# SomeBottle/LinearProgramming

Measured on AMD Instinct MI355X. Metric: Simplex pivots/sec + HBM GB/s fraction, dense m=16384×n=32768 fp64, 1/2/4/8 GPU, higher is better.
Workload: dtype f64

## Files before the change

include/lpg.h:

```cpp
#ifndef LPG_H
#define LPG_H

#include <stddef.h>
#include <stdint.h>

#ifdef __cplusplus
extern "C" {
#endif

#define LPG_OK           0
#define LPG_ERR_ARG     -1
#define LPG_ERR_DEVICE  -2
#define LPG_ERR_OOM     -3
#define LPG_ERR_STATE   -4
#define LPG_ERR_COMM    -5

#define LPG_RUNNING      0
#define LPG_OPTIMAL      1
#define LPG_UNBOUNDED    2
#define LPG_INFEASIBLE   3
#define LPG_ITER_LIMIT   4
#define LPG_NUMERIC      5

#define LPG_RULE_DANTZIG 0
// ... 23 lines not shown
} lpg_result;

typedef struct {
    int64_t m, ncols, ld;
    int64_t row0, nrows;
    int32_t world, rank, device;
    int32_t nobj;
    int32_t defer_k;
    int32_t pivot_wg;
    double  bytes_per_pivot;
    int32_t exchange;
    int32_t column_trade;
    int32_t residency_fallbacks;
    int32_t region;
    int32_t region_recoveries;
} lpg_info_t;

typedef struct {
    double  update_ms;
    double  select_ms;
    double  comm_ms;
    int64_t update_count;
    double  update_bytes;
} lpg_timing;

typedef struct {
    void *user;
    int (*allgather)(void *user, const void *send, void *recv, size_t bytes_per_rank);
    int (*allreduce_sum_f64)(void *user, double *buf, size_t count);
} lpg_host_comm_ops;
// ... 145 lines not shown
```

linearprogramming_amd/_lib.py:

```python
from __future__ import annotations

import ctypes
import os
import sys

_HERE = os.path.dirname(os.path.abspath(__file__))
LIB_PATH = os.path.join(_HERE, "liblpg.so")

OK, ERR_ARG, ERR_DEVICE, ERR_OOM, ERR_STATE, ERR_COMM = 0, -1, -2, -3, -4, -5
RUNNING, OPTIMAL, UNBOUNDED, INFEASIBLE, ITER_LIMIT, NUMERIC = 0, 1, 2, 3, 4, 5
STATUS_NAMES = {0: "RUNNING", 1: "OPTIMAL", 2: "UNBOUNDED", 3: "INFEASIBLE", 4: "ITER_LIMIT", 5: "NUMERIC"}
RULE_DANTZIG, RULE_BLAND = 0, 1
GEN_DENSE, GEN_DEGENERATE, GEN_ARTIFICIAL, GEN_DUAL = 0, 1, 2, 3
FLAG_NO_LOG = 0x1
FLAG_NO_SKIP = 0x2
FLAG_BIG_M = 0x4
FLAG_EAGER = 0x8
DEFER_MAX = 128
BATCH_TIER_LDS, BATCH_TIER_GLOBAL = 0, 1
BATCH_MAX_DIM = 8192
BRANCH_MOST_FRACTIONAL, BRANCH_FIRST = 0, 1
BATCH_MAX_CUTS = 1024

c_double_p = ctypes.POINTER(ctypes.c_double)
# ... 2 lines not shown
c_int8_p = ctypes.POINTER(ctypes.c_int8)


class Result(ctypes.Structure):
    _fields_ = [("status", ctypes.c_int32), ("rule", ctypes.c_int32), ("pivots", ctypes.c_int64),
                ("objective", ctypes.c_double), ("entering", ctypes.c_int64), ("leaving", ctypes.c_int64)]


class Info(ctypes.Structure):
    _fields_ = [("m", ctypes.c_int64), ("ncols", ctypes.c_int64), ("ld", ctypes.c_int64),
                ("row0", ctypes.c_int64), ("nrows", ctypes.c_int64),
                ("world", ctypes.c_int32), ("rank", ctypes.c_int32), ("device", ctypes.c_int32),
                ("nobj", ctypes.c_int32), ("defer_k", ctypes.c_int32), ("pivot_wg", ctypes.c_int32),
                ("bytes_per_pivot", ctypes.c_double), ("exchange", ctypes.c_int32), ("column_trade", ctypes.c_int32),
                ("residency_fallbacks", ctypes.c_int32), ("region", ctypes.c_int32),
                ("region_recoveries", ctypes.c_int32)]


class Timing(ctypes.Structure):
    _fields_ = [("update_ms", ctypes.c_double), ("select_ms", ctypes.c_double),
                ("comm_ms", ctypes.c_double), ("update_count", ctypes.c_int64), ("update_bytes", ctypes.c_double)]


class BatchInfo(ctypes.Structure):
    _fields_ = [("count", ctypes.c_int64), ("m", ctypes.c_int64), ("ncols", ctypes.c_int64), ("ld", ctypes.c_int64),
                ("tier", ctypes.c_int32), ("chunk", ctypes.c_int32), ("lds_bytes", ctypes.c_int64),
                ("log_capacity", ctypes.c_int64), ("nobj", ctypes.c_int32), ("pad", ctypes.c_int32)]


class BatchShape(ctypes.Structure):
    _fields_ = [("m", ctypes.c_int64), ("ncols", ctypes.c_int64), ("ld", ctypes.c_int64),
# ... 219 lines not shown
```

linearprogramming_amd/csrc/lpg_block.hip:

```cpp
#include <hip/hip_runtime.h>
#include <math.h>
#include <stdint.h>

#include <algorithm>
#include <atomic>

#include "lpg_device.h"
#include "lpg_internal.h"

namespace lpg {

typedef unsigned u4 __attribute__((ext_vector_type(4)));

namespace {

constexpr int kNT = 256;
constexpr int kMaxWG = 256;
constexpr int kPer = kMaxWG / 64;
constexpr int kRecPMax = 5;
constexpr int kRecR = 2;
constexpr int kMaxLds = 150 * 1024;
constexpr long long kSpinTicks = 200000000ll;
constexpr int kSweepSleep = 1;

// ... 347 lines not shown
    int ncin;
    Xch X;
    uint32_t xtag0;
    const double *Cs0;
    double *Cs1;
    Defer D;
    u4 *rec;
    uint32_t tag0;
    int nwg, cw, rw, ks;
    uint32_t cl;
    int xcd1;
    const int32_t *live;
    int64_t nlive;
    const int64_t *bcol0;
    int nsp, cwx;
};

template <int RULE, int NOBJ, bool MR, int KB, bool REG>
__global__ __launch_bounds__(kNT, 1) void k_pivot_block(BlockArgs a) {
    static_assert(!REG || NOBJ == 1, "region mode: one objective row");
    constexpr bool B2 = KB > 64;
    constexpr int WS = B2 ? 104 : 72;
    constexpr bool KDR = RULE != RULE_BLAND && NOBJ == 1;
    constexpr int GDR = KDR ? 0 : 2;
    constexpr int NGP = 2 + (KDR ? 0 : 1) + (NOBJ == 2 ? 1 : 0);
    constexpr bool RPIV = !MR && RULE != RULE_BLAND;
    constexpr int NGR = RPIV ? 1 : kRecR;
    static_assert(NGP < kRecPMax, "pricing records (nwg * NGP + 1 granules) exceed their reservation");
    constexpr bool PK1 = NOBJ == 1;
    constexpr bool PKD = PK1 && !KDR;
// ... 400 lines not shown
                }
                if (hc) pq = __longlong_as_double((long long)ld_sys64(xch_row(a.X, a.X.rank, xpar, owner, g.ld) + c));
            }
            if (wg == 0 && tid == 0) {
                D.lv[q] = lvv;
                D.basis[r] = kt;
            }
        }
        if (REG && actnow) {
            pql = (MR && !own) ? __longlong_as_double((long long)ld_sys64(xch_row(a.X, a.X.rank, xpar, xowner, g.ld) +
                                                                          (uint32_t)bc0))
                               : x / piv;
            sPt[q] = pql;
            cobl = cobjR;
            actq = q;
        }
        if (hc) {
            sPt[q] = pq;
            st_wt(D.Pbuf + (int64_t)q * g.ld + c, pq);
            if (NOBJ == 2) dM = fma(-cobjM, pq, dM);
            dR = fma(-cobjR, pq, dR);
            price_one<RULE>(pb, dM, dR, lj, g, c);
            pb.pad = (int32_t)c;
        }
        LPG_BPH(t, 10);
        pb = block_argmin_pp<RULE, kNT / 64, false>(pb);
        LPG_BPH(t, 11);
        if (tid == 0) {
            uint64_t h = ~0ull;
            uint32_t l = ~0u;
            if (pb.j >= 0) {
                h = RULE == RULE_BLAND ? 0ull
                                       : (((uint64_t)(uint32_t)pb.cls << 63) |
                                          (~(uint64_t)__double_as_longlong(pb.v) & 0x7fffffffffffffffull));
// ... 401 lines not shown
    hipLaunchKernelGGL(k_region_build, dim3(1), dim3(1024), 0, (hipStream_t)L.stream, st, basis, inv, g.m, g.ncols,
                       g.ld, mark, live, bcol0, nlive, tlive);
    return hipGetLastError() == hipSuccess ? 0 : -1;
}

int launch_region_check(const Launch &L, const Geo &g, const int64_t *basis, const int32_t *inv, int *ok) {
    const int64_t rows = g.nloc + g.nobj;
    hipLaunchKernelGGL(k_region_check, dim3((unsigned)((rows + 63) / 64), (unsigned)((g.m + 255) / 256)), dim3(256), 0,
                       (hipStream_t)L.stream, g.T, g, basis, inv, ok);
    return hipGetLastError() == hipSuccess ? 0 : -1;
}

int launch_pivot_block(const Launch &L, const Geo &g, int rule, DevState *st, int s0, int q0, int n, Cand *part,
                       int ncand, const Cand *cin, int ncin, const double *Cs0, double *Cs1, const Defer &D,
                       void *rec, uint32_t tag0, int nwg, int cw, int rw, int ks, size_t lds, uint32_t cl,
                       const Xch *X, uint32_t xtag0, const RegionArgs *R) {
    if (n < 1 || q0 < 0 || q0 + n > ks || ks > 96 || nwg < 1 || nwg > kMaxWG || ncand < nwg || cl < 1) return -1;
    if (X && (X->world < 1 || X->world > 64 || X->nblk < nwg || X->nx < 1)) return -1;
    if (!R && ((int64_t)nwg * cw < ((g.ncols + 1) & ~(int64_t)1) || (int64_t)nwg * rw < g.nloc)) return -1;
    if (R && (g.nobj != 1 || (int64_t)nwg * cw < R->nlive || (int64_t)nwg * rw < g.nloc ||
              (int64_t)nwg * R->nsp < ks || R->cwx != cw + R->nsp + 1 || R->cwx > kNT || !R->live || !R->bcol0))
        return -1;
    if (g.nobj != 1 && g.nobj != 2) return -1;
    BlockArgs a;
    a.T = g.T;
    a.g = g;
    a.st = st;
    a.s0 = s0;
    a.q0 = q0;
    a.n = n;
    a.part = part;
// ... 5 lines not shown
    a.Cs0 = Cs0;
    a.Cs1 = Cs1;
    a.D = D;
    a.rec = (u4 *)rec;
    a.tag0 = tag0;
    a.nwg = nwg;
    a.cw = cw;
    a.rw = rw;
    a.ks = ks;
    a.cl = cl;
    a.live = R ? R->live : nullptr;
    a.nlive = R ? R->nlive : 0;
    a.bcol0 = R ? R->bcol0 : nullptr;
    a.nsp = R ? R->nsp : 0;
    a.cwx = R ? R->cwx : cw;
    hipStream_t stream = (hipStream_t)L.stream;
    static const bool xcd1_on = [] {
        const char *e = getenv("LPG_PIVOT_XCD1");
        return !(e && e[0] == '0');
    }();

    int dev = 0;
    if (hipGetDevice(&dev) != hipSuccess || dev < 0 || dev >= 64) return -1;
    static std::atomic<int> cus_of[64];
    int cus = cus_of[dev].load(std::memory_order_relaxed);
    if (cus == 0) {
        if (hipDeviceGetAttribute(&cus, hipDeviceAttributeMultiprocessorCount, dev) != hipSuccess) cus = -1;
        cus_of[dev].store(cus, std::memory_order_relaxed);
    }
    a.xcd1 = (xcd1_on && !X && cus >= 8 * 32 && nwg <= cus / 8) ? 1 : 0;
// ... 44 lines not shown
```

linearprogramming_amd/csrc/lpg_ctx.hip:

```cpp
#include <hip/hip_runtime.h>
#include <rccl/rccl.h>

#include <dlfcn.h>
#include <unistd.h>
#include <math.h>
#include <stdarg.h>
#include <stdio.h>
#include <stdlib.h>
#include <string.h>

#include <algorithm>
#include <cmath>
#include <vector>

#include "../../include/lpg.h"
#include "lpg_internal.h"

using namespace lpg;

namespace {

thread_local char g_err[512];

struct TimingRing {
// ... 37 lines not shown
    int skip_cfg = 1;
    bool no_reorder_cfg = false;
    bool signed_zeros = false;
    bool nonfinite = false;
    int pb_nwg = 0, pb_cw = 0, pb_rw = 0;
    size_t pb_lds = 0;
    bool reg = false;
    bool reg_valid = false;
    bool units_known = false;
    RegionGeo rg{};
    int32_t *live = nullptr, *mark = nullptr;
    int32_t *tlive = nullptr;
    bool block_region = false;
    bool tlive_on = true;
    bool move_unit = true;
    int64_t *bcol0 = nullptr;
    int *rok = nullptr;
    void *rec = nullptr;
    uint32_t tag = 0;
    uint32_t pb_launch = 0;
    int64_t lost = 0;
    int res_fallbacks = 0;
    int reg_recoveries = 0;
    char *xbuf = nullptr;
    int64_t xbytes = 0, xoffF = 0, xoffC = 0, xoffG = 0;
    int xnblk = 0, xnx = 0;
    bool xuncached = false;
    char **xbase = nullptr;
    std::vector<void *> xpeer;
    bool xmode = false;
// ... 231 lines not shown
        default: break;
    }
    return 0;
}

#endif

static int flush_launch(lpg_ctx *c) {
    int rc;
    const bool re = reorders(c);
#ifdef LPG_TEST_HOOKS
    if (c->inject_flush >= 0 && c->nflush == c->inject_flush && (rc = inject_pending_fault(c))) return rc;
#endif
    c->nflush++;
    const int unit = (c->block_region && c->reg_valid && c->move_unit) ? 1 : 0;
    if (launch_swap_plan(lau(c), geo(c), c->st, defer_of(c, 0), c->colmap, c->inv, c->pairs, re ? 1 : 0, c->defer_k) ||
        (re && launch_move_cols(lau(c), geo(c), c->st, defer_of(c, 0), c->pairs, unit)))
        return fail(c, LPG_ERR_DEVICE, "swap plan launch failed");
#ifdef LPG_TEST_HOOKS
    if (c->inject_rbad >= 0 && c->nflush == c->inject_rbad + 1)
        HIPCHK(c, hipMemsetAsync(&c->st->rbad, 0x01, sizeof(uint32_t), c->stream));
#endif
    if (c->timing && ((rc = timing_mark(c, 0)) || (rc = timing_mark(c, 1)))) return rc;
    const int32_t *tl = (c->block_region && c->reg_valid && re && c->tlive_on && c->skip) ? c->tlive : nullptr;
    c->block_region = false;
    if (launch_flush_main(lau(c), geo(c), c->st, defer_of(c, 0), c->pend, c->skip, c->flush_variant, c->flush_xcd, tl))
        return fail(c, LPG_ERR_DEVICE, "flush launch failed");
    if (c->timing && (rc = timing_mark(c, 2, 2))) return rc;
    if (launch_flush_tail(lau(c), geo(c), c->st, defer_of(c, 0), c->pend, !re))
        return fail(c, LPG_ERR_DEVICE, "flush launch failed");
    if (re) {
        const Defer D = defer_of(c, 0);
        if (launch_fill_cols(lau(c), geo(c), c->pairs, c->st, &D, flush_kmax_supported(c->defer_k),
                             c->reg ? c->bcol0 : nullptr))
            return fail(c, LPG_ERR_DEVICE, "fill launch failed");
        c->permuted = true;
    }
    c->pend = 0;
    return 0;
}

static int materialize(lpg_ctx *c) {
    if (c->defer_k == 0 || c->pend == 0) return 0;
    return flush_launch(c);
// ... 179 lines not shown
        if (mr) {
            ncand = std::max(ncand, nwg);
            ncin = c->x_from_cand ? cand_per_rank(c) * c->world : nwg;
            if (c->x_from_cand) cin = c->cand;
            X.base = c->xbase;
            X.world = c->world;
            X.rank = c->rank;
            X.nblk = c->xnblk;
            X.nx = c->xnx;
            X.from_cand = 0;
            X.tag = c->xtag;
            X.offF = c->xoffF;
            X.offC = c->xoffC;
            X.offG = c->xoffG;
        }
        const bool ok = reg ? launch_pivot_block(lau(c), g, rule, c->st, s0, c->pend, n, c->part, ncand, cin, ncin,
                                                 c->C[s0], c->C[s1], defer_of(c, c->pend), c->rec, c->tag, c->rg.nwg,
                                                 c->rg.cw, c->rg.rw, c->defer_k, c->rg.lds, c->pb_launch + 1,
                                                 mr ? &X : nullptr, c->xtag, &R) == 0
                            : launch_pivot_block(lau(c), g, rule, c->st, s0, c->pend, n, c->part, ncand, cin, ncin,
                                                 c->C[s0], c->C[s1], defer_of(c, c->pend), c->rec, c->tag, c->pb_nwg,
                                                 c->pb_cw, c->pb_rw, c->defer_k, c->pb_lds, c->pb_launch + 1,
                                                 mr ? &X : nullptr, c->xtag) == 0;
        if (!ok)
            return fail(c, LPG_ERR_DEVICE, "pivot block launch failed");
        if (reg) c->block_region = true;
        c->pb_launch++;
        if (mr) {
            c->xtag += (uint32_t)n;
            c->x_from_cand = false;
        }
        c->tag += (uint32_t)n;
        c->pend += n;
        c->par = s1;
        c->enq += n;
        npiv -= n;
        if (c->pend == c->defer_k) {
            int rc = flush_launch(c);
            if (rc) return rc;
        }
    }
// ... 178 lines not shown
    return 0;
}

static int recover_region(lpg_ctx *c, const DevState &h) {
    c->reg_recoveries++;
    c->lost += std::max<int64_t>(c->enq - h.pivots, 0);
    c->enq = h.pivots;
    c->pend = (int)h.npend;
    c->booted = false;
    c->reg_valid = false;
    HIPCHK(c, hipMemsetAsync(&c->st->stall, 0, sizeof(int64_t), c->stream));
    return 0;
}

static int pending_fault(lpg_ctx *c, const DevState &h) {
    static const char *const what[] = {"?", "npend", "kq", "lv", "rq"};
    const int64_t w = h.stall_info[0] >= 1 && h.stall_info[0] <= 4 ? h.stall_info[0] : 0;
    c->poisoned = true;
    return fail(c, LPG_ERR_STATE,
                "pending block inconsistent at the flush (%s[%lld] = %lld, npend %lld): the loop was stopped with "
                "NUMERIC instead of indexing with it; the constraint rows were not brought up to date",
                what[w], (long long)h.stall_info[1], (long long)h.stall_info[2], (long long)h.stall_info[3]);
}

static int usable(lpg_ctx *c) {
    if (!c->poisoned) return 0;
    return fail(c, LPG_ERR_STATE, "context unusable: an earlier flush refused an inconsistent pending block, so the "
                "basis and the constraint rows disagree; reload the rows and the basis (lpg_load_rows, lpg_set_basis) or "
                "regenerate (lpg_generate) the LP");
}

static int read_result(lpg_ctx *c, lpg_result *out, int rule) {
// ... 34 lines not shown
    }
    return 0;
}

static int reset_state(lpg_ctx *c) {
    DevState h;
    memset(&h, 0, sizeof h);
    h.logcap = c->logcap;
    h.last_k = h.last_r = -1;
    HIPCHK(c, hipMemcpyAsync(c->st, &h, sizeof h, hipMemcpyHostToDevice, c->stream));
    HIPCHK(c, hipStreamSynchronize(c->stream));
    c->booted = false;
    c->par = 0;
    c->enq = 0;
    c->pend = 0;
    c->touched_mark = 0;
    c->pb_launch = 0;
    c->lost = 0;
    return 0;
}

static void graph_drop(lpg_ctx *c);

static int ensure_log(lpg_ctx *c, int64_t need) {
    if (c->flags & LPG_FLAG_NO_LOG) return 0;
    if (need <= c->logcap) return 0;
    graph_drop(c);
    int64_t cap = std::max<int64_t>(need, 2 * c->logcap);
    int64_t *nk = nullptr, *nr = nullptr;
    HIPCHK(c, hipStreamSynchronize(c->stream));
// ... 107 lines not shown
            static const char *const names[] = {"", "npend", "kq", "lv", "rq", "ahead"};
            for (int u = 1; u <= 5; u++)
                if (!strcmp(w, names[u])) c->inject_what = u;
            c->inject_flush = c->inject_what ? f : -1;
        }
    }
    if (const char *rb = getenv("LPG_TEST_REGION_BAD")) c->inject_rbad = atoi(rb);
#endif
    const char *fv = getenv("LPG_FLUSH_KERNEL");
    c->flush_variant = fv ? (fv[0] == 'w' ? 1 : fv[0] == 'm' ? 0 : -1) : -1;
    const char *ft = getenv("LPG_FLUSH_TLIVE");
    c->tlive_on = !(ft && ft[0] == '0');
    {
        const char *mu = getenv("LPG_MOVE_UNIT");
        c->move_unit = !(mu && mu[0] == '0');
    }
    const char *fx = getenv("LPG_FLUSH_XCD");
    c->flush_xcd = -1;
    if (fx && fx[0] == '0') c->flush_xcd = 0;
    if (fx && fx[0] == '1') c->flush_xcd = 1;
    if (fx && fx[0] == 'h' && (fx[1] == '1' || fx[1] == '2' || fx[1] == '4' || fx[1] == '8')) c->flush_xcd = 10 + (fx[1] - '0');
    int rc;
    if ((rc = use_device(c))) { lpg_destroy(c); return rc; }
    const int64_t rows = c->nloc + c->nobj;
    const Geo g = geo(c);
    c->npp = price_blocks(g);
    const int64_t maxloc = (m + world - 1) / world + c->nobj;
    c->nsel = (int)std::min<int64_t>((maxloc + kBlock - 1) / kBlock, kMaxSelBlocks);
    c->npp_d = pivot_d_blocks(g, 0, c->pivot_nt);
    c->nsel_d = world == 1 ? pivot_d_blocks(g, 1, c->pivot_nt) : (int)((maxloc + 255) / 256);
// ... 308 lines not shown
    o->row0 = c->row0;
    o->nrows = c->nloc;
    o->world = c->world;
    o->rank = c->rank;
    o->device = c->device;
    o->nobj = (int32_t)c->nobj;
    o->defer_k = c->defer_k;
    const bool pb = (c->persist && !has_comm(c)) || (c->persist_x && c->xmode);
    o->pivot_wg = pb ? (c->reg ? c->rg.nwg : c->pb_nwg) : 0;
    o->bytes_per_pivot = 16.0 * (double)(c->nloc + c->nobj) * (double)c->ncols;
    o->exchange = c->xmode ? (c->xuncached ? 2 : 1) : 0;
    o->column_trade = reorders(c) ? 1 : 0;
    o->residency_fallbacks = c->res_fallbacks;
    o->region_recoveries = c->reg_recoveries;
    o->region = (o->pivot_wg > 0 && c->reg) ? 1 : 0;
    return 0;
}

int lpg_load_rows(lpg_ctx *c, int64_t row0, int64_t nrows, const double *rows, int64_t ld) {
    if (!c || !rows || row0 < 0 || nrows < 0 || row0 + nrows > c->m + c->nobj || ld < c->ncols)
        return fail(c, LPG_ERR_ARG, "lpg_load_rows: bad arguments");
    int rc;
    if ((rc = use_device(c)) || (rc = canonicalize(c))) return rc;
    {
        bool sz = false, nf = false;
        for (int64_t i = 0; i < nrows; i++) {
            const double *row = rows + i * ld;
            for (int64_t j = 0; j < c->ncols; j++) {
                const double v = row[j];
                nf |= !std::isfinite(v);
// ... 91 lines not shown
    c->nact = nact;
    c->booted = false;
    graph_drop(c);
    return 0;
}

int lpg_generate(lpg_ctx *c, int64_t n, uint64_t seed, int kind) {
    if (!c || n < 1 || c->ncols != n + c->m + 1 || kind < LPG_GEN_DENSE || kind > LPG_GEN_DUAL)
        return fail(c, LPG_ERR_ARG, "lpg_generate: need ncols == n + m + 1 and a known kind");
    int rc;
    if ((rc = use_device(c))) return rc;
    if (c->colmap && (launch_iota(lau(c), c->colmap, c->ld) || launch_iota(lau(c), c->inv, c->ld)))
        return fail(c, LPG_ERR_DEVICE, "iota launch failed");
    c->permuted = false;
    c->pend = 0;
    if (launch_generate(lau(c), geo(c), n, seed, kind, c->basis)) return fail(c, LPG_ERR_DEVICE, "generate launch failed");
    c->poisoned = false;
    c->units_known = true;
    c->signed_zeros = c->nonfinite = false;
    HIPCHK(c, hipStreamSynchronize(c->stream));
    return reset_state(c);
}

int lpg_enqueue(lpg_ctx *c, int64_t npiv, int rule) {
    if (!c || npiv < 0 || (rule != LPG_RULE_DANTZIG && rule != LPG_RULE_BLAND))
        return fail(c, LPG_ERR_ARG, "lpg_enqueue: bad arguments");
    int rc;
    if ((rc = use_device(c))) return rc;
    if ((rc = usable(c))) return rc;
    if ((rc = ensure_log(c, c->enq + npiv))) return rc;
// ... 77 lines not shown
    c->lost = 0;
    if ((rc = materialize(c))) return rc;
    return read_result(c, out, rule);
}

int lpg_pivot(lpg_ctx *c, int64_t k, int64_t r) {
    if (!c || k < 1 || k >= c->ncols || r < 0 || r >= c->m) return fail(c, LPG_ERR_ARG, "lpg_pivot: bad (k, r)");
    int rc;
    if ((rc = use_device(c))) return rc;
    if ((rc = usable(c))) return rc;
    if ((rc = ensure_log(c, c->enq + 1))) return rc;
    const int rule = c->booted ? c->boot_rule : LPG_RULE_DANTZIG;
    lpg_result before, after;
    if ((rc = read_result(c, &before, rule))) return rc;
    if ((rc = bootstrap_forced(c, rule, k, r))) return rc;
    if ((rc = enqueue(c, 1, rule))) return rc;
    if ((rc = read_result(c, &after, rule))) return rc;
    c->booted = false;
    if (after.pivots != before.pivots + 1)
        return fail(c, LPG_ERR_STATE, "lpg_pivot: |T[%lld][%lld]| <= eps_piv, pivot not applied", (long long)r, (long long)k);
    return 0;
}

static int host_allreduce_sum(lpg_ctx *c, double *v, size_t count) {
    if (!has_comm(c)) return 0;
    if (count > (size_t)c->ncols) return fail(c, LPG_ERR_ARG, "host_allreduce_sum: %zu > ncols", count);
    HIPCHK(c, hipMemcpyAsync(c->acc, v, count * sizeof(double), hipMemcpyHostToDevice, c->stream));
    int rc;
    if ((rc = comm_allreduce_sum(c, c->acc, count))) return rc;
    HIPCHK(c, hipMemcpyAsync(v, c->acc, count * sizeof(double), hipMemcpyDeviceToHost, c->stream));
// ... 362 lines not shown
```

linearprogramming_amd/csrc/lpg_internal.h:

```cpp
#pragma once
#include <stddef.h>
#include <stdint.h>

namespace lpg {

constexpr int kBlock = 256;
constexpr int kMaxSelBlocks = 512;
#ifndef LPG_DEFER_MAX
#define LPG_DEFER_MAX 128
#endif

enum : int32_t { RUNNING = 0, OPTIMAL = 1, UNBOUNDED = 2, INFEASIBLE = 3, ITER_LIMIT = 4, NUMERIC = 5 };
enum : int { RULE_DANTZIG = 0, RULE_BLAND = 1 };

struct Slot {
    int64_t k;
    int64_t r;
    int32_t status;
    int32_t pad0;
    int64_t dpend;
};

struct DevState {
    Slot    slot[2];
// ... 112 lines not shown
    size_t lds;
};
struct RegionArgs {
    const int32_t *live;
    int64_t nlive;
    const int64_t *bcol0;
    int nsp, cwx;
};
int block_geometry_region(const Geo &g, int ks, int cus, int want, int64_t nlive, RegionGeo *out);
int launch_region_build(const Launch &L, const Geo &g, DevState *st, const int64_t *basis, const int32_t *inv,
                        int32_t *mark, int32_t *live, int64_t *bcol0, int64_t nlive, int32_t *tlive);
int launch_region_check(const Launch &L, const Geo &g, const int64_t *basis, const int32_t *inv, int *ok);
int launch_pivot_block(const Launch &L, const Geo &g, int rule, DevState *st, int s0, int q0, int n, Cand *part,
                       int ncand, const Cand *cin, int ncin, const double *Cs0, double *Cs1, const Defer &D,
                       void *rec, uint32_t tag0, int nwg, int cw, int rw, int ks, size_t lds, uint32_t cl,
                       const Xch *X = nullptr, uint32_t xtag0 = 0, const RegionArgs *R = nullptr);
int launch_flush(const Launch &L, const Geo &g, DevState *st, const Defer &D, int kmax, int skip, int which);
int launch_flush_main(const Launch &L, const Geo &g, DevState *st, const Defer &D, int kmax, int skip, int which,
                      int xcd = -1, const int32_t *tlive = nullptr);
int launch_flush_tail(const Launch &L, const Geo &g, DevState *st, const Defer &D, int kmax, bool reset = true);
__host__ __device__ inline int64_t flush_tail_rows(int64_t rows, int64_t nloc) {
    return (rows > 0 && nloc >= 8 * rows && rows >= 64) ? rows / 4 : 0;
}
__host__ __device__ inline int64_t flush_nitems(int64_t ntiles, int64_t rows, int64_t nloc) {
    const int64_t tr = flush_tail_rows(rows, nloc);
    if (rows < 0) rows = -rows;
    if (!tr) return ntiles * ((nloc + rows - 1) / rows);
    const int64_t t0 = ((nloc + rows - 1) / rows - 2) * rows;
    return ntiles * (t0 / rows) + ntiles * ((nloc - t0 + tr - 1) / tr);
}
__host__ __device__ inline void flush_item(int64_t item, int64_t ntiles, int64_t rows, int64_t nloc, int64_t &tile,
                                           int64_t &i0, int64_t &i1) {
    const int64_t tr = flush_tail_rows(rows, nloc);
    if (rows < 0) rows = -rows;
    const int64_t t0 = tr ? ((nloc + rows - 1) / rows - 2) * rows : nloc;
// ... 54 lines not shown
    } else if (it - full < G.ntg - G.ttg) {
        j = G.ntg - 1 - (it - full);
        i0 = base;
        i1 = G.r1;
    } else {
        const int64_t k = it - full - (G.ntg - G.ttg);
        j = G.ttg - 1 - k / G.nq;
        i0 = base + (k % G.nq) * G.qrows;
        i1 = i0 + G.qrows;
    }
    if (i1 > G.r1) i1 = G.r1;
    tile = h + (int64_t)f.H * j;
}
int flush_kmax_supported(int k);
int launch_swap_plan(const Launch &L, const Geo &g, DevState *st, const Defer &D, int32_t *colmap, int32_t *inv,
                     int32_t *pairs, int plan, int kmax);
constexpr int kPairW = 4;
int launch_move_cols(const Launch &L, const Geo &g, const DevState *st, const Defer &D, const int32_t *pairs,
                     int unit);
int launch_fill_cols(const Launch &L, const Geo &g, const int32_t *pairs, DevState *st = nullptr,
                     const Defer *D = nullptr, int kmax = 0, int64_t *bcol0 = nullptr);
int launch_gather_rows(const Launch &L, const Geo &g, const int32_t *inv, double *tmp, int64_t i0, int64_t nr);
int launch_iota(const Launch &L, int32_t *a, int64_t n);
int launch_update(const Launch &L, const Geo &g, DevState *st, int s, const double *P, const double *Cs,
                  int64_t *basis, int64_t *logk, int64_t *logr, int variant, int skip);

int launch_dual_rows(const Launch &L, const Geo &g, Cand *part, int nsel);
int launch_dual_row_d(const Launch &L, const Geo &g, DevState *st, int s, const Cand *rc, int nrc, Cand *cp,
                      double *R, const double *Pprev, const double *Cprev, const Defer &D, bool mr);
int launch_dual_ratio(const Launch &L, const Geo &g, const DevState *st, int s, const double *R, Cand *cp);
int launch_dual_col_d(const Launch &L, const Geo &g, DevState *st, int s, const Cand *cp, const double *R, double *Cs,
                      Cand *rc, int nrc_out, const Defer &D);
int launch_dual_pivot(const Launch &L, const Geo &g, DevState *st, int s, Cand *part, int nsel, PricePart *pp,
                      int *pc, int npp, int skip, double *P, double *Cs, bool price_only = false);
// ... 11 lines not shown
```

linearprogramming_amd/csrc/lpg_kernels.hip:

```cpp
#include <hip/hip_runtime.h>
#include <math.h>

#include <stddef.h>
#include <stdlib.h>

#include <algorithm>

#include "lpg_internal.h"
#include "lpg_device.h"
#include "lpg_flushw.h"

namespace lpg {



static inline uint64_t splitmix64_host(uint64_t x) {
    uint64_t z = x + 0x9E3779B97F4A7C15ull;
    z = (z ^ (z >> 30)) * 0xBF58476D1CE4E5B9ull;
    z = (z ^ (z >> 27)) * 0x94D049BB133111EBull;
    return z ^ (z >> 31);
}
static inline uint64_t subkey(uint64_t seed, uint64_t which) {
    return splitmix64_host(seed ^ (which * 0xD1B54A32D192ED03ull));
}
// ... 1647 lines not shown
            if (q >= np) break;
            const int64_t r = q < 64 ? (int64_t)rdl64((uint64_t)ru, q) : (int64_t)rdl64((uint64_t)ru1, q - 64);
            if (r < 0) continue;
            if (__ballot(c > q && ru == r)) continue;
            if (K > 64 && __ballot(64 + c > q && ru1 == r)) continue;
            if (ok) T[r * g.ld + j] = xs[i];
        }
    }
}


constexpr int kMulBlocks = 8;
constexpr int kPlanNT = LPG_DEFER_MAX;
__global__ __launch_bounds__(kPlanNT) void k_swap_plan(DevState *__restrict__ st, const int64_t *__restrict__ kq,
                                                  const int64_t *__restrict__ lv, const int64_t *__restrict__ rq,
                                                  const double *__restrict__ Cbuf, int64_t cs,
                                                  int32_t *__restrict__ colmap, int32_t *__restrict__ inv,
                                                  int32_t *__restrict__ pairs, double *__restrict__ mul, int plan,
                                                  const double *__restrict__ pv, int64_t nloc, int64_t ncols, int kmax) {
    const int64_t np64 = st->npend;
    const bool npbad = np64 < 0 || np64 > kmax;
    const int np = npbad ? 0 : (int)np64;
    {
        const int q = threadIdx.x;
        int what = npbad ? 1 : 0;
        int64_t val = np64;
        if (!npbad && q < np) {
            const int64_t x = plan ? kq[q] : 1, y = plan ? lv[q] : 1, r = rq[q];
            if (x < 1 || x >= ncols) what = 2, val = x;
            else if (y < 1 || y >= ncols) what = 3, val = y;
            else if (r < -1 || r >= nloc) what = 4, val = r;
        }
        __shared__ int first;
        if (q == 0) first = kPlanNT;
        __syncthreads();
        if (what) atomicMin(&first, q);
        if (__syncthreads_or(what != 0)) {
            if (blockIdx.x == 0 && q == first) {
                if (st->stall == 0) {
                    st->stall_info[0] = what;
                    st->stall_info[1] = q;
                    st->stall_info[2] = val;
                    st->stall_info[3] = np64;
                    st->stall = kStallPending;
                }
                st->npend = 0;
                if (pairs) pairs[0] = 0;
                for (int u = 0; u < 2; u++)
                    if (st->slot[u].status == RUNNING) st->slot[u].status = NUMERIC;
            }
            return;
        }
    }
    if (blockIdx.x > 0) {
        constexpr int UB = LPG_DEFER_MAX / kMulBlocks;
        const int q = threadIdx.x;
        const int u0 = (blockIdx.x - 1) * UB;
        const int64_t r = q < np ? rq[q] : -1;
        double v[UB];
#pragma unroll
        for (int k = 0; k < UB; k++) {
            const int u = u0 + k;
            const bool on = u > q && u < np && r >= 0;
            const double c = Cbuf[(int64_t)(on ? u : 0) * cs + (on ? r : 0)];
            v[k] = on ? -c : 0.0;
        }
#pragma unroll
        for (int k = 0; k < UB; k++)
            if (u0 + k < np) mul[(u0 + k) * LPG_DEFER_MAX + q] = v[k];
        return;
    }
    if (!plan) return;
    const int q = threadIdx.x;
// ... 55 lines not shown
        const int32_t a = inv[ce], b = inv[cl];
        pairs[1 + kPairW * q] = a;
        pairs[2 + kPairW * q] = b;
        pairs[3 + kPairW * q] = (int32_t)eR[q];
        pairs[4 + kPairW * q] = (int32_t)eRL[q];
        colmap[a] = (int32_t)cl;
        colmap[b] = (int32_t)ce;
        inv[cl] = a;
        inv[ce] = b;
    }
    if (q == 0) pairs[0] = n;
}

__global__ __launch_bounds__(kBlock) void k_move_cols(double *__restrict__ T, Geo g, const DevState *__restrict__ st,
                                                      double *__restrict__ Pbuf, const int32_t *__restrict__ pairs,
                                                      int npb, int unit) {
    const int n = pairs[0];
    if (n == 0) return;
    const int nrb = (int)gridDim.x - npb;
    if ((int)blockIdx.x >= nrb) {
        const int np = (int)st->npend;
        const int nt = npb * (int)gridDim.y * kBlock;
        for (int e = (((int)blockIdx.x - nrb) * (int)gridDim.y + (int)blockIdx.y) * kBlock + threadIdx.x; e < np * n;
             e += nt) {
            const int q = e / n, p = e - q * n;
            double *Pq = Pbuf + (int64_t)q * g.ld;
            const int32_t a = pairs[1 + kPairW * p], b = pairs[2 + kPairW * p];
            Pq[a] = Pq[b];
            Pq[b] = 0.0;
        }
        return;
    }
    const int64_t i = (int64_t)blockIdx.x * kBlock + threadIdx.x;
    if (i >= g.nloc + g.nobj) return;
    const bool obj = i >= g.nloc;
    double *row = T + i * g.ld;
    for (int p0 = 16 * blockIdx.y; p0 < n; p0 += 16 * gridDim.y) {
        double va[16], vb[16];
        int ia[16], ib[16], rl[16];
#pragma unroll
        for (int u = 0; u < 16; u++) {
            ia[u] = p0 + u < n ? pairs[1 + kPairW * (p0 + u)] : 0;
            ib[u] = p0 + u < n ? pairs[2 + kPairW * (p0 + u)] : 0;
            rl[u] = p0 + u < n ? pairs[4 + kPairW * (p0 + u)] : -1;
        }
#pragma unroll
        for (int u = 0; u < 16; u++) {
            vb[u] = (unit && !obj) ? ((int64_t)rl[u] == i ? 1.0 : 0.0) : row[ib[u]];
            va[u] = obj ? row[ia[u]] : 0.0;
        }
// ... 40 lines not shown
    if (bcol0 && blockIdx.y == 0) {
        for (int64_t r = (int64_t)blockIdx.x * kBlock + threadIdx.x; r < g.m; r += (int64_t)gridDim.x * kBlock) {
            const int64_t v = D.basis[r];
            bcol0[r] = (v << 32) | (int64_t)(uint32_t)D.inv[v];
        }
    }
    const int n = pairs[0];
    const int64_t i = (int64_t)blockIdx.x * kBlock + threadIdx.x;
    if (i >= g.nloc || n == 0) return;
    double *row = T + i * g.ld;
    for (int p = blockIdx.y; p < n; p += gridDim.y)
        row[pairs[2 + kPairW * p]] = (i == (int64_t)pairs[3 + kPairW * p]) ? 1.0 : 0.0;
}

int launch_swap_plan(const Launch &L, const Geo &g, DevState *st, const Defer &D, int32_t *colmap, int32_t *inv,
                     int32_t *pairs, int plan, int kmax) {
    kmax = flush_kmax_supported(kmax);
    if (!kmax || (plan && !pairs)) return -1;
    hipLaunchKernelGGL(k_swap_plan, dim3(1 + kMulBlocks), dim3(kPlanNT), 0, (hipStream_t)L.stream, st, D.kq, D.lv, D.rq,
                       D.Cbuf, D.cs, colmap, inv, pairs, D.mul, plan, D.pv, g.nloc, g.ncols, kmax);
    return hipGetLastError() == hipSuccess ? 0 : -1;
}

int launch_move_cols(const Launch &L, const Geo &g, const DevState *st, const Defer &D, const int32_t *pairs,
                     int unit) {
    const int64_t rows = g.nloc + g.nobj;
    const int npb = (LPG_DEFER_MAX * LPG_DEFER_MAX + 4 * kBlock - 1) / (4 * kBlock);
    hipLaunchKernelGGL(k_move_cols, dim3((unsigned)((rows + kBlock - 1) / kBlock + npb), 4), dim3(kBlock), 0,
                       (hipStream_t)L.stream, g.T, g, st, D.Pbuf, pairs, npb, unit);
    return hipGetLastError() == hipSuccess ? 0 : -1;
}

int launch_fill_cols(const Launch &L, const Geo &g, const int32_t *pairs, DevState *st, const Defer *D, int kmax,
                     int64_t *bcol0) {
    if (st && (!D || !D->rq || kmax < 1 || kmax > LPG_DEFER_MAX)) return -1;
    if (bcol0 && (!st || !D->basis || !D->inv || !D->lv || !D->Pbuf)) return -1;
    hipLaunchKernelGGL(k_fill_cols, dim3((unsigned)std::max<int64_t>((g.nloc + kBlock - 1) / kBlock, 1), 4), dim3(kBlock),
                       0, (hipStream_t)L.stream, g.T, g, pairs, st, D ? *D : Defer{}, kmax, bcol0);
    return hipGetLastError() == hipSuccess ? 0 : -1;
}

__global__ __launch_bounds__(kBlock) void k_gather_rows(const double *__restrict__ T, Geo g,
                                                        const int32_t *__restrict__ inv, double *__restrict__ tmp,
                                                        int64_t i0, int64_t nr) {
// ... 23 lines not shown
}

int flush_kmax_supported(int k) {
    if (k <= 8) return 8;
    if (k <= 16) return 16;
    if (k <= 32) return 32;
    if (k <= 64) return 64;
    if (k <= 96) return 96;
    if (k <= 128 && k <= LPG_DEFER_MAX) return 128;
    return 0;
}

static_assert(offsetof(DevState, fwork) == offsetof(DevState, npend) + sizeof(int64_t),
              "launch_flush clears npend and fwork with one memset");

int launch_flush_tail(const Launch &L, const Geo &g, DevState *st, const Defer &D, int kmax, bool reset) {
    kmax = flush_kmax_supported(kmax);
    if (!kmax) return -1;
    hipStream_t stream = (hipStream_t)L.stream;
    const int64_t ntiles_p = (g.ncols + 63) / 64;
#ifdef LPG_PIVROWS96
    if (kmax == 96)
        hipLaunchKernelGGL(k_flush_pivot_rows<96>, dim3((unsigned)ntiles_p), dim3(kBlock), 0, stream, g.T, g, st,
                           D.Pbuf, D.mul, D.rq);
    else
#endif
    if (kmax > 64)
        hipLaunchKernelGGL(k_flush_pivot_rows<128>, dim3((unsigned)ntiles_p), dim3(kBlock), 0, stream, g.T, g, st,
                           D.Pbuf, D.mul, D.rq);
    else
        hipLaunchKernelGGL(k_flush_pivot_rows<64>, dim3((unsigned)ntiles_p), dim3(kBlock), 0, stream, g.T, g, st,
                           D.Pbuf, D.mul, D.rq);
    if (hipGetLastError() != hipSuccess) return -1;
    if (!reset) return 0;
// ... 144 lines not shown
```

Measured before the change: 31260.

## Write pivot rows directly during the pivot block to skip the pivot-row flush pass

Single-device, non-exchange pivot blocks now write the normalized pivot row straight into the tableau as it is computed (seed mode). When every pending pivot in a block was seeded, the flush skips the separate k_flush_pivot_rows pass and only zeroes the matching column-buffer entries. It also keeps pivot rows out of the unit move in k_move_cols, and adds a validity check on the pivot values. This removes one full read/write pass over the pivot rows per flush, at the cost of extra stores inside the pivot kernel and added state tracking (seeded_pend, block_forced).

Result: no change. 31820 (median of 3 runs) (+1.8%).

```diff
diff --git a/include/lpg.h b/include/lpg.h
--- a/include/lpg.h
+++ b/include/lpg.h
@@ -61,6 +61,7 @@
     int32_t residency_fallbacks;
     int32_t region;
     int32_t region_recoveries;
+    int32_t rows_in_pass;
 } lpg_info_t;
 
 typedef struct {
diff --git a/linearprogramming_amd/_lib.py b/linearprogramming_amd/_lib.py
--- a/linearprogramming_amd/_lib.py
+++ b/linearprogramming_amd/_lib.py
@@ -40,7 +40,7 @@
                 ("nobj", ctypes.c_int32), ("defer_k", ctypes.c_int32), ("pivot_wg", ctypes.c_int32),
                 ("bytes_per_pivot", ctypes.c_double), ("exchange", ctypes.c_int32), ("column_trade", ctypes.c_int32),
                 ("residency_fallbacks", ctypes.c_int32), ("region", ctypes.c_int32),
-                ("region_recoveries", ctypes.c_int32)]
+                ("region_recoveries", ctypes.c_int32), ("rows_in_pass", ctypes.c_int32)]
 
 
 class Timing(ctypes.Structure):
diff --git a/linearprogramming_amd/csrc/lpg_block.hip b/linearprogramming_amd/csrc/lpg_block.hip
--- a/linearprogramming_amd/csrc/lpg_block.hip
+++ b/linearprogramming_amd/csrc/lpg_block.hip
@@ -385,6 +385,7 @@
     int64_t nlive;
     const int64_t *bcol0;
     int nsp, cwx;
+    int seed;
 };
 
 template <int RULE, int NOBJ, bool MR, int KB, bool REG>
@@ -815,10 +816,12 @@
             sPt[q] = pql;
             cobl = cobjR;
             actq = q;
+            if (!MR && a.seed) st_wt(g.T + rl * g.ld + (int64_t)(uint32_t)bc0, pql);
         }
         if (hc) {
             sPt[q] = pq;
             st_wt(D.Pbuf + (int64_t)q * g.ld + c, pq);
+            if (!MR && a.seed) st_wt(g.T + rl * g.ld + c, pq);
             if (NOBJ == 2) dM = fma(-cobjM, pq, dM);
             dR = fma(-cobjR, pq, dR);
             price_one<RULE>(pb, dM, dR, lj, g, c);
@@ -1250,7 +1253,8 @@
 int launch_pivot_block(const Launch &L, const Geo &g, int rule, DevState *st, int s0, int q0, int n, Cand *part,
                        int ncand, const Cand *cin, int ncin, const double *Cs0, double *Cs1, const Defer &D,
                        void *rec, uint32_t tag0, int nwg, int cw, int rw, int ks, size_t lds, uint32_t cl,
-                       const Xch *X, uint32_t xtag0, const RegionArgs *R) {
+                       const Xch *X, uint32_t xtag0, const RegionArgs *R, int seed) {
+    if (seed && X) return -1;
     if (n < 1 || q0 < 0 || q0 + n > ks || ks > 96 || nwg < 1 || nwg > kMaxWG || ncand < nwg || cl < 1) return -1;
     if (X && (X->world < 1 || X->world > 64 || X->nblk < nwg || X->nx < 1)) return -1;
     if (!R && ((int64_t)nwg * cw < ((g.ncols + 1) & ~(int64_t)1) || (int64_t)nwg * rw < g.nloc)) return -1;
@@ -1286,6 +1290,7 @@
     a.bcol0 = R ? R->bcol0 : nullptr;
     a.nsp = R ? R->nsp : 0;
     a.cwx = R ? R->cwx : cw;
+    a.seed = seed ? 1 : 0;
     hipStream_t stream = (hipStream_t)L.stream;
     static const bool xcd1_on = [] {
         const char *e = getenv("LPG_PIVOT_XCD1");
diff --git a/linearprogramming_amd/csrc/lpg_ctx.hip b/linearprogramming_amd/csrc/lpg_ctx.hip
--- a/linearprogramming_amd/csrc/lpg_ctx.hip
+++ b/linearprogramming_amd/csrc/lpg_ctx.hip
@@ -75,6 +75,10 @@
     bool block_region = false;
     bool tlive_on = true;
     bool move_unit = true;
+    bool pivrows_pass = true;
+    int seeded_pend = 0;
+    bool block_forced = false;
+    int rows_in_pass = 0;
     int64_t *bcol0 = nullptr;
     int *rok = nullptr;
     void *rec = nullptr;
@@ -336,8 +340,14 @@
 #endif
     c->nflush++;
     const int unit = (c->block_region && c->reg_valid && c->move_unit) ? 1 : 0;
-    if (launch_swap_plan(lau(c), geo(c), c->st, defer_of(c, 0), c->colmap, c->inv, c->pairs, re ? 1 : 0, c->defer_k) ||
-        (re && launch_move_cols(lau(c), geo(c), c->st, defer_of(c, 0), c->pairs, unit)))
+    const bool ride = c->pivrows_pass && c->pend > 0 && c->seeded_pend >= c->pend && !c->block_forced &&
+                      c->world == 1 && !has_comm(c) && !c->signed_zeros && !c->nonfinite;
+    c->seeded_pend = 0;
+    c->block_forced = false;
+    if (ride) c->rows_in_pass++;
+    if (launch_swap_plan(lau(c), geo(c), c->st, defer_of(c, 0), c->colmap, c->inv, c->pairs, re ? 1 : 0, c->defer_k,
+                         ride ? 1 : 0) ||
+        (re && launch_move_cols(lau(c), geo(c), c->st, defer_of(c, 0), c->pairs, unit, ride ? 1 : 0)))
         return fail(c, LPG_ERR_DEVICE, "swap plan launch failed");
 #ifdef LPG_TEST_HOOKS
     if (c->inject_rbad >= 0 && c->nflush == c->inject_rbad + 1)
@@ -349,7 +359,7 @@
     if (launch_flush_main(lau(c), geo(c), c->st, defer_of(c, 0), c->pend, c->skip, c->flush_variant, c->flush_xcd, tl))
         return fail(c, LPG_ERR_DEVICE, "flush launch failed");
     if (c->timing && (rc = timing_mark(c, 2, 2))) return rc;
-    if (launch_flush_tail(lau(c), geo(c), c->st, defer_of(c, 0), c->pend, !re))
+    if (launch_flush_tail(lau(c), geo(c), c->st, defer_of(c, 0), c->pend, !re, !ride))
         return fail(c, LPG_ERR_DEVICE, "flush launch failed");
     if (re) {
         const Defer D = defer_of(c, 0);
@@ -559,17 +569,20 @@
             X.offC = c->xoffC;
             X.offG = c->xoffG;
         }
+        const int seed = (c->pivrows_pass && !mr && c->world == 1 && !c->block_forced && !c->signed_zeros &&
+                          !c->nonfinite && c->seeded_pend >= c->pend) ? 1 : 0;
         const bool ok = reg ? launch_pivot_block(lau(c), g, rule, c->st, s0, c->pend, n, c->part, ncand, cin, ncin,
                                                  c->C[s0], c->C[s1], defer_of(c, c->pend), c->rec, c->tag, c->rg.nwg,
                                                  c->rg.cw, c->rg.rw, c->defer_k, c->rg.lds, c->pb_launch + 1,
-                                                 mr ? &X : nullptr, c->xtag, &R) == 0
+                                                 mr ? &X : nullptr, c->xtag, &R, seed) == 0
                             : launch_pivot_block(lau(c), g, rule, c->st, s0, c->pend, n, c->part, ncand, cin, ncin,
                                                  c->C[s0], c->C[s1], defer_of(c, c->pend), c->rec, c->tag, c->pb_nwg,
                                                  c->pb_cw, c->pb_rw, c->defer_k, c->pb_lds, c->pb_launch + 1,
-                                                 mr ? &X : nullptr, c->xtag) == 0;
+                                                 mr ? &X : nullptr, c->xtag, nullptr, seed) == 0;
         if (!ok)
             return fail(c, LPG_ERR_DEVICE, "pivot block launch failed");
         if (reg) c->block_region = true;
+        if (seed) c->seeded_pend += n;
         c->pb_launch++;
         if (mr) {
             c->xtag += (uint32_t)n;
@@ -778,8 +791,8 @@
 }
 
 static int pending_fault(lpg_ctx *c, const DevState &h) {
-    static const char *const what[] = {"?", "npend", "kq", "lv", "rq"};
-    const int64_t w = h.stall_info[0] >= 1 && h.stall_info[0] <= 4 ? h.stall_info[0] : 0;
+    static const char *const what[] = {"?", "npend", "kq", "lv", "rq", "pv bits"};
+    const int64_t w = h.stall_info[0] >= 1 && h.stall_info[0] <= 5 ? h.stall_info[0] : 0;
     c->poisoned = true;
     return fail(c, LPG_ERR_STATE,
                 "pending block inconsistent at the flush (%s[%lld] = %lld, npend %lld): the loop was stopped with "
@@ -844,6 +857,8 @@
     c->par = 0;
     c->enq = 0;
     c->pend = 0;
+    c->seeded_pend = 0;
+    c->block_forced = false;
     c->touched_mark = 0;
     c->pb_launch = 0;
     c->lost = 0;
@@ -981,6 +996,8 @@
     {
         const char *mu = getenv("LPG_MOVE_UNIT");
         c->move_unit = !(mu && mu[0] == '0');
+        const char *pr = getenv("LPG_PIVROWS_PASS");
+        c->pivrows_pass = !(pr && pr[0] == '0');
     }
     const char *fx = getenv("LPG_FLUSH_XCD");
     c->flush_xcd = -1;
@@ -1319,6 +1336,7 @@
     o->residency_fallbacks = c->res_fallbacks;
     o->region_recoveries = c->reg_recoveries;
     o->region = (o->pivot_wg > 0 && c->reg) ? 1 : 0;
+    o->rows_in_pass = c->rows_in_pass;
     return 0;
 }
 
@@ -1440,6 +1458,8 @@
         return fail(c, LPG_ERR_DEVICE, "iota launch failed");
     c->permuted = false;
     c->pend = 0;
+    c->seeded_pend = 0;
+    c->block_forced = false;
     if (launch_generate(lau(c), geo(c), n, seed, kind, c->basis)) return fail(c, LPG_ERR_DEVICE, "generate launch failed");
     c->poisoned = false;
     c->units_known = true;
@@ -1547,6 +1567,7 @@
     lpg_result before, after;
     if ((rc = read_result(c, &before, rule))) return rc;
     if ((rc = bootstrap_forced(c, rule, k, r))) return rc;
+    c->block_forced = true;
     if ((rc = enqueue(c, 1, rule))) return rc;
     if ((rc = read_result(c, &after, rule))) return rc;
     c->booted = false;
diff --git a/linearprogramming_amd/csrc/lpg_internal.h b/linearprogramming_amd/csrc/lpg_internal.h
--- a/linearprogramming_amd/csrc/lpg_internal.h
+++ b/linearprogramming_amd/csrc/lpg_internal.h
@@ -150,11 +150,12 @@
 int launch_pivot_block(const Launch &L, const Geo &g, int rule, DevState *st, int s0, int q0, int n, Cand *part,
                        int ncand, const Cand *cin, int ncin, const double *Cs0, double *Cs1, const Defer &D,
                        void *rec, uint32_t tag0, int nwg, int cw, int rw, int ks, size_t lds, uint32_t cl,
-                       const Xch *X = nullptr, uint32_t xtag0 = 0, const RegionArgs *R = nullptr);
+                       const Xch *X = nullptr, uint32_t xtag0 = 0, const RegionArgs *R = nullptr, int seed = 0);
 int launch_flush(const Launch &L, const Geo &g, DevState *st, const Defer &D, int kmax, int skip, int which);
 int launch_flush_main(const Launch &L, const Geo &g, DevState *st, const Defer &D, int kmax, int skip, int which,
                       int xcd = -1, const int32_t *tlive = nullptr);
-int launch_flush_tail(const Launch &L, const Geo &g, DevState *st, const Defer &D, int kmax, bool reset = true);
+int launch_flush_tail(const Launch &L, const Geo &g, DevState *st, const Defer &D, int kmax, bool reset = true,
+                      bool rewrite = true);
 __host__ __device__ inline int64_t flush_tail_rows(int64_t rows, int64_t nloc) {
     return (rows > 0 && nloc >= 8 * rows && rows >= 64) ? rows / 4 : 0;
 }
@@ -239,10 +240,10 @@
 }
 int flush_kmax_supported(int k);
 int launch_swap_plan(const Launch &L, const Geo &g, DevState *st, const Defer &D, int32_t *colmap, int32_t *inv,
-                     int32_t *pairs, int plan, int kmax);
+                     int32_t *pairs, int plan, int kmax, int ride = 0);
 constexpr int kPairW = 4;
 int launch_move_cols(const Launch &L, const Geo &g, const DevState *st, const Defer &D, const int32_t *pairs,
-                     int unit);
+                     int unit, int ride = 0);
 int launch_fill_cols(const Launch &L, const Geo &g, const int32_t *pairs, DevState *st = nullptr,
                      const Defer *D = nullptr, int kmax = 0, int64_t *bcol0 = nullptr);
 int launch_gather_rows(const Launch &L, const Geo &g, const int32_t *inv, double *tmp, int64_t i0, int64_t nr);
diff --git a/linearprogramming_amd/csrc/lpg_kernels.hip b/linearprogramming_amd/csrc/lpg_kernels.hip
--- a/linearprogramming_amd/csrc/lpg_kernels.hip
+++ b/linearprogramming_amd/csrc/lpg_kernels.hip
@@ -1685,10 +1685,11 @@
 constexpr int kPlanNT = LPG_DEFER_MAX;
 __global__ __launch_bounds__(kPlanNT) void k_swap_plan(DevState *__restrict__ st, const int64_t *__restrict__ kq,
                                                   const int64_t *__restrict__ lv, const int64_t *__restrict__ rq,
-                                                  const double *__restrict__ Cbuf, int64_t cs,
+                                                  double *__restrict__ Cbuf, int64_t cs,
                                                   int32_t *__restrict__ colmap, int32_t *__restrict__ inv,
                                                   int32_t *__restrict__ pairs, double *__restrict__ mul, int plan,
-                                                  const double *__restrict__ pv, int64_t nloc, int64_t ncols, int kmax) {
+                                                  const double *__restrict__ pv, int64_t nloc, int64_t ncols, int kmax,
+                                                  int ride) {
     const int64_t np64 = st->npend;
     const bool npbad = np64 < 0 || np64 > kmax;
     const int np = npbad ? 0 : (int)np64;
@@ -1701,6 +1702,7 @@
             if (x < 1 || x >= ncols) what = 2, val = x;
             else if (y < 1 || y >= ncols) what = 3, val = y;
             else if (r < -1 || r >= nloc) what = 4, val = r;
+            else if (ride && !(pv[q] > 0.0 && pv[q] <= 1.79769313486231570e308)) what = 5, val = (int64_t)__double_as_longlong(pv[q]);
         }
         __shared__ int first;
         if (q == 0) first = kPlanNT;
@@ -1728,6 +1730,16 @@
         const int q = threadIdx.x;
         const int u0 = (blockIdx.x - 1) * UB;
         const int64_t r = q < np ? rq[q] : -1;
+        if (ride) {
+            __shared__ int64_t sr[kPlanNT];
+            sr[q] = r;
+            __syncthreads();
+            bool lastq = r >= 0;
+            for (int u = q + 1; u < np; u++) lastq = lastq && sr[u] != r;
+            if (lastq)
+                for (int u = u0; u < u0 + UB && u <= q; u++) Cbuf[(int64_t)u * cs + r] = 0.0;
+            return;
+        }
         double v[UB];
 #pragma unroll
         for (int k = 0; k < UB; k++) {
@@ -1813,7 +1825,7 @@
 
 __global__ __launch_bounds__(kBlock) void k_move_cols(double *__restrict__ T, Geo g, const DevState *__restrict__ st,
                                                       double *__restrict__ Pbuf, const int32_t *__restrict__ pairs,
-                                                      int npb, int unit) {
+                                                      int npb, int unit, const int64_t *__restrict__ rq) {
     const int n = pairs[0];
     if (n == 0) return;
     const int nrb = (int)gridDim.x - npb;
@@ -1833,6 +1845,12 @@
     const int64_t i = (int64_t)blockIdx.x * kBlock + threadIdx.x;
     if (i >= g.nloc + g.nobj) return;
     const bool obj = i >= g.nloc;
+    if (unit && rq && !obj) {
+        const int np = (int)st->npend;
+        bool prow = false;
+        for (int q = 0; q < np; q++) prow = prow || rq[q] == i;
+        if (prow) unit = 0;
+    }
     double *row = T + i * g.ld;
     for (int p0 = 16 * blockIdx.y; p0 < n; p0 += 16 * gridDim.y) {
         double va[16], vb[16];
@@ -1903,20 +1921,20 @@
 }
 
 int launch_swap_plan(const Launch &L, const Geo &g, DevState *st, const Defer &D, int32_t *colmap, int32_t *inv,
-                     int32_t *pairs, int plan, int kmax) {
+                     int32_t *pairs, int plan, int kmax, int ride) {
     kmax = flush_kmax_supported(kmax);
     if (!kmax || (plan && !pairs)) return -1;
     hipLaunchKernelGGL(k_swap_plan, dim3(1 + kMulBlocks), dim3(kPlanNT), 0, (hipStream_t)L.stream, st, D.kq, D.lv, D.rq,
-                       D.Cbuf, D.cs, colmap, inv, pairs, D.mul, plan, D.pv, g.nloc, g.ncols, kmax);
+                       D.Cbuf, D.cs, colmap, inv, pairs, D.mul, plan, D.pv, g.nloc, g.ncols, kmax, ride);
     return hipGetLastError() == hipSuccess ? 0 : -1;
 }
 
 int launch_move_cols(const Launch &L, const Geo &g, const DevState *st, const Defer &D, const int32_t *pairs,
-                     int unit) {
+                     int unit, int ride) {
     const int64_t rows = g.nloc + g.nobj;
     const int npb = (LPG_DEFER_MAX * LPG_DEFER_MAX + 4 * kBlock - 1) / (4 * kBlock);
     hipLaunchKernelGGL(k_move_cols, dim3((unsigned)((rows + kBlock - 1) / kBlock + npb), 4), dim3(kBlock), 0,
-                       (hipStream_t)L.stream, g.T, g, st, D.Pbuf, pairs, npb, unit);
+                       (hipStream_t)L.stream, g.T, g, st, D.Pbuf, pairs, npb, unit, ride ? D.rq : nullptr);
     return hipGetLastError() == hipSuccess ? 0 : -1;
 }
 
@@ -1970,10 +1988,15 @@
 static_assert(offsetof(DevState, fwork) == offsetof(DevState, npend) + sizeof(int64_t),
               "launch_flush clears npend and fwork with one memset");
 
-int launch_flush_tail(const Launch &L, const Geo &g, DevState *st, const Defer &D, int kmax, bool reset) {
+int launch_flush_tail(const Launch &L, const Geo &g, DevState *st, const Defer &D, int kmax, bool reset, bool rewrite) {
     kmax = flush_kmax_supported(kmax);
     if (!kmax) return -1;
     hipStream_t stream = (hipStream_t)L.stream;
+    if (!rewrite) {
+        if (!reset) return 0;
+        hipLaunchKernelGGL(k_end_block, dim3(1), dim3(kBlock), 0, stream, st, D, kmax);
+        return hipGetLastError() == hipSuccess ? 0 : -1;
+    }
     const int64_t ntiles_p = (g.ncols + 63) / 64;
 #ifdef LPG_PIVROWS96
     if (kmax == 96)
```
